# PhucNguyenAH/tacotron2_subword

Hardware: AMD Instinct MI355X
Metric: mel_frames_per_sec_train (higher is better)
Workload: dtype bf16; 1 GPU; BERT_Tacotron2 default hparams (SMA), full training iteration fwd+loss+bwd+clip+Adam, B=64/GPU, 100 phones, 60 sub-word tokens, 400 frames, 80-mel; global_batch=64, frames_per_item=400, parallelism=dp1, torch_ops=loss reductions, cat/transpose copies, persistent_chains=True, recurrent_steps_bf16=True

## Files before the change

### tacotron2_subword_amd/csrc/chain.hip

```cpp
#include <algorithm>
#include <cstdlib>
#include <type_traits>

#include "chain_common.h"

#ifdef T2_STAMPS
__device__ unsigned long long t2_chain_stamps[256 * 16];
extern "C" int t2_debug_read_chain_stamps(unsigned long long* out, int n) {
    return (int)hipMemcpyFromSymbol(out, HIP_SYMBOL(t2_chain_stamps), sizeof(unsigned long long) * n);
}
extern "C" int t2_debug_clear_chain_stamps(void) {
    static unsigned long long z[256 * 16];
    return (int)hipMemcpyToSymbol(HIP_SYMBOL(t2_chain_stamps), z, sizeof(z));
}
#define T2_CSTAMP(i)                                                                              \
    do {                                                                                          \
        __builtin_amdgcn_sched_barrier(0);                                                        \
        if (threadIdx.x == 0) { const unsigned long long n_ = __builtin_amdgcn_s_memrealtime(); t2_stamp_lds[i] += n_ - stamp_last; stamp_last = n_; } \
        __builtin_amdgcn_sched_barrier(0);                                                        \
    } while (0)
#else
#define T2_CSTAMP(i)
#endif

// ... 285 lines not shown
            }
        }
#endif
    };
    auto store_A_saved = [&](int t, int tid) {
        if (DEC) return;
#ifndef T2_CHAIN_NOSAVE
        const long rb = (long)t * B + ab_;
        for (int c = tid; c < EC; c += NTH) {
            const float x = csL[c];
            d.din[rb * d.WD + AS.coff + c0 + c] = x;
            d.dout[rb * d.WO + AS.ctx2off + c0 + c] = x;
            d.din16[rb * d.WD + AS.coff + c0 + c] = (__bf16)x;
        }
        if (KIND == CHAIN_LSA && AS.locsave) {
            const int F = d.F, DP = F + 8;
            float* ls = AS.locsave + rb * Tin * F;
            for (int i = tid; i < Tin * (F / 4); i += NTH) {
                const int j = i / (F / 4), f4 = (i % (F / 4)) * 4;
                if (j % d.CS != part) continue;
                const bf16x4 hi = *reinterpret_cast<const bf16x4*>(lspL + j * DP + f4), lo = *reinterpret_cast<const bf16x4*>(lspL + (Tin + j) * DP + f4);
                __builtin_nontemporal_store(f32x4{(float)hi[0] + (float)lo[0], (float)hi[1] + (float)lo[1], (float)hi[2] + (float)lo[2], (float)hi[3] + (float)lo[3]},
                                            reinterpret_cast<f32x4*>(ls + j * F + f4));
            }
        }
#endif
    };
#ifdef T2_STAMPS
    __shared__ __attribute__((aligned(16))) unsigned long long t2_stamp_lds[16];
    if (threadIdx.x < 16) t2_stamp_lds[threadIdx.x] = 0;
    __syncthreads();
    unsigned long long stamp_last = __builtin_amdgcn_s_memrealtime();
#endif
    for (int t = d.t0; t < d.t1; ++t) {
        const unsigned ep = (unsigned)(t - d.t0);
        const bool more = t + 1 < d.t1;
        int tv = threadIdx.x;
        asm volatile("" : "+v"(tv));
        const unsigned xout = (unsigned)((t & 1) * d.NS) * G.xs_bytes;
        if (hasL) {
            float pre[NSLOT][4];
#pragma unroll
            for (int sl = 0; sl < NSLOT; ++sl)
#pragma unroll
                for (int g = 0; g < 4; ++g) pre[sl][g] = pre_next[sl][g];
            T2_CSTAMP(15);
            if (DEC) {
                if (wave == 0 && !poll_counter(cntH_L, ep, (unsigned)G.NUG, d.err, 1u) && lane == 0) *abortw = 1;
                __syncthreads();
                if (*abortw) return;
            }
            T2_CSTAMP(0);
            if (EARLY) issue_h(t - 1);
            if (DEC) {
                if (wave == 0) {
                    bool ok = poll_counter(cntC_L, ep, nA_per_step, d.err, 2u);
                    if (ok) ok = poll_counter(d.cnt + (size_t)(10 + ls) * CNT_STRIDE, ep, (unsigned)(d.P / 16), d.err, 11u);
                    if (!ok && lane == 0) *abortw = 1;
                }
                __syncthreads();
                if (*abortw) return;
            }
            T2_CSTAMP(2);
            if (EARLY) mfma_h(t - 1);
#pragma unroll
            for (int rt = 0; rt < RT; ++rt) {
                if (!EARLY) { zero_acc(); gemm_part(t - 1, rt, wave * KH, 0, std::integral_constant<int, KH>{}); }
                if (KC > 0) gemm_part(t - 1, rt, H / 16 + wave * KC, KH, std::integral_constant<int, KC>{});
                if (DEC) gemm_part(t - 1, rt, (H + d.E) / 16 + wave * KPN, KH + KC, std::integral_constant<int, KPN>{});
                T2_CSTAMP(14);
#pragma unroll
                for (int ut = 0; ut < UT; ++ut) {
                    const int tp = rt * UT + ut;
                    if (tp > 0) __syncthreads();
#pragma unroll
                    for (int e = 0; e < 16; ++e)
                        partL[(wave * 32 + (e & 3) + 8 * (e >> 2) + 4 * hk) * PPR + r] = acc[ut][e];
                    __syncthreads();
                    if ((tid >> 8) == (tp & 1)) {
                        const int sl = tp >> 1;
                        const int bl = (tid & 255) >> 3, uu = tid & 7;
                        const int b = row0 + rt * 32 + bl, u = u0 + ut * 8 + uu;
                        float g4[4];
#pragma unroll
                        for (int g = 0; g < 4; ++g) {
                            float sum = 0.f;
#pragma unroll
                            for (int w = 0; w < NWV; ++w) sum += partL[(w * 32 + bl) * PPR + g * 8 + uu];
                            g4[g] = sum + pre[sl][g];
                        }
                        const float ig = fast_sigmoid(g4[0]), fg = fast_sigmoid(g4[1]), gg = fast_tanh(g4[2]), og = fast_sigmoid(g4[3]);
                        const float cn = fg * cst[sl] + ig * gg;
                        const float hn = og * fast_tanh(cn);
                        float ho = hn, co = cn;
                        if (d.drop_p > 0.f) {
                            const uint32_t idx = (uint32_t)(((long)t * B + b) * H + u);
                            ho = rng_keep(kh, idx, d.drop_p) ? hn * dscale : 0.f;
                            co = rng_keep(kc, idx, d.drop_p) ? cn * dscale : 0.f;
                        }
                        if (b >= B) { ho = 0.f; co = 0.f; }
                        cst[sl] = co;
                        sv[sl][0] = ig; sv[sl][1] = fg; sv[sl][2] = gg; sv[sl][3] = og; sv[sl][4] = cn; sv[sl][5] = co; sv[sl][6] = ho;
                        hsL[(rt * 32 + bl) * HSP + ut * 8 + uu] = ho;
                    }
                }
            }
            __syncthreads();
            T2_CSTAMP(3);
            if (wave < RT && rg * RT + wave < G.MT) {
                const int rtg = rg * RT + wave;
                if (UT == 2 || hk == 0) {
                    const int kh8 = UT == 2 ? hk : ((u0 >> 3) & 1);
                    const float* hp = hsL + (wave * 32 + r) * HSP + (UT == 2 ? hk * 8 : 0);
                    const f32x4 lo = *reinterpret_cast<const f32x4*>(hp), hi = *reinterpret_cast<const f32x4*>(hp + 4);
                    bf16x8 o;
#pragma unroll
                    for (int j = 0; j < 4; ++j) { o[j] = (__bf16)lo[j]; o[4 + j] = (__bf16)hi[j]; }
                    u32x4 ow = __builtin_bit_cast(u32x4, o);
                    if (!DEC) ow.x = (ow.x & ~1u) | step_tag(t);
                    __builtin_amdgcn_raw_buffer_store_b128(ow, rsX,
                        xout + (unsigned)ls * G.xs_bytes + (unsigned)((((u0 >> 4) * G.MT + rtg) * 64 + kh8 * 32 + r) * 16), 0, SC1);
                }
            }
            if (KIND != CHAIN_LSTM) {
                if (wave < 4 * RT) {
                    const int ct = wave & 3, rt = wave >> 2;
                    f32x16 qa;
#pragma unroll
                    for (int e = 0; e < 16; ++e) qa[e] = 0.f;
#pragma unroll
                    for (int m = 0; m < UT * 4; ++m)
                        qa = __builtin_amdgcn_mfma_f32_32x32x2f32(hsL[(rt * 32 + r) * HSP + 2 * m + hk], wqf[m], qa, 0, 0, 0);
#pragma unroll
                    for (int e = 0; e < 16; ++e) qsL[(rt * 32 + (e & 3) + 8 * (e >> 2) + 4 * hk) * (A + 4) + ct * 32 + r] = qa[e];
                }
                __syncthreads();
                const unsigned qb = (unsigned)(((ls * G.NRG + rg) * G.NUG + ug) * (32 * RT)) * (unsigned)(A * 4);
                for (int i = tv; i < RT * 32 * (A / 4); i += NTH) {
                    const int row = i / (A / 4), a4 = (i % (A / 4)) * 4;
                    const f32x4 v4 = *reinterpret_cast<const f32x4*>(qsL + row * (A + 4) + a4);
                    u32x4 vw = __builtin_bit_cast(u32x4, v4);
                    vw.x = (vw.x & ~1u) | tag_q(t);
                    __builtin_amdgcn_raw_buffer_store_b128(vw, rsQ, qb + (unsigned)((row * A + a4) * 4), 0, SC1);
                }
            }
            T2_CSTAMP(4);
            if (DEC) publish(cntH_L, (unsigned)ug); else { __syncthreads(); if (*abortw) return; }
            T2_CSTAMP(5);
            store_L_saved(t, tv);
            if (!DEC && !hasA && more) load_pre(t + 1, tv);
        }
        if (hasA) {
            const int tid = tv, lane = tid & 63, wave = tid >> 6;
            T2_CSTAMP(6);
            if (KIND == CHAIN_LSA) {
                const int F = d.F, Kc = d.Kc, pad = (Kc - 1) / 2, Tw = Tin + Kc - 1, TwP = (Tw + 8 + 3) & ~3, KP = (Kc + 7) & ~7, WP = 2 * KP + 8;
                for (int i = tid; i < 2 * TwP; i += NTH) {
                    const int c = i / TwP, j = i % TwP - pad;
                    wpadL[i] = (j >= 0 && j < Tin) ? (c == 0 ? apL[j] : cumL[j]) : 0.f;
                }
                __syncthreads();
                const int r_ = lane & 31, h_ = lane >> 5;
                const int njt = (Tin + 31) / 32, nft = (F + 31) / 32;
                for (int tile = wave; tile < njt * nft; tile += NWV) {
                    const int jt = tile / nft, ft = tile % nft;
                    const float* xr = wpadL + min(jt * 32 + r_, Tin - 1);
                    const __bf16* wh = convwL + min(ft * 32 + r_, F - 1) * WP + 8 * h_;
                    f32x16 acc;
#pragma unroll
                    for (int e2 = 0; e2 < 16; ++e2) acc[e2] = 0.f;
                    for (int k0 = 0; k0 < 2 * KP; k0 += 16) {
                        const int ck = k0 + 8 * h_, c = ck >= KP ? 1 : 0;
                        const float* xp = xr + c * TwP + ck - c * KP;
                        float xv[8];
#pragma unroll
                        for (int u = 0; u < 8; ++u) xv[u] = xp[u];
                        bf16x8 ah, al;
#pragma unroll
                        for (int u = 0; u < 8; ++u) { ah[u] = (__bf16)xv[u]; al[u] = (__bf16)(xv[u] - (float)ah[u]); }
                        const bf16x8 bh = *reinterpret_cast<const bf16x8*>(wh + k0), bl = *reinterpret_cast<const bf16x8*>(wh + F * WP + k0);
                        acc = __builtin_amdgcn_mfma_f32_32x32x16_bf16(al, bh, acc, 0, 0, 0);
                        acc = __builtin_amdgcn_mfma_f32_32x32x16_bf16(ah, bl, acc, 0, 0, 0);
                        acc = __builtin_amdgcn_mfma_f32_32x32x16_bf16(ah, bh, acc, 0, 0, 0);
                    }
                    const int f = ft * 32 + r_;
                    if (f < F) {
#pragma unroll
                        for (int e2 = 0; e2 < 16; ++e2) {
                            const int row = jt * 32 + (e2 & 3) + 8 * (e2 >> 2) + 4 * h_;
                            if (row < Tin) {
                                const float x = acc[e2];
                                const __bf16 hi = (__bf16)x;
                                lspL[row * (F + 8) + f] = hi; lspL[(Tin + row) * (F + 8) + f] = (__bf16)(x - (float)hi);
                            }
                        }
                    }
                }
            }
            if (KIND == CHAIN_LSA) __syncthreads();
            if (*abortw) return;
            T2_CSTAMP(7);
            {
                const int pg = tid >> 5, a4 = (tid & 31) * 4;
                const unsigned qb = (unsigned)((as * G.NRG + arg) * G.NUG) * (unsigned)(32 * RT * A * 4) + (unsigned)((arow * A + a4) * 4);
                constexpr int QU = 4;
                u32x4 pv[QU];
                auto load_q = [&](int i0) {
                    const unsigned long long tsp = __builtin_amdgcn_s_memrealtime();
                    for (;;) {
                        unsigned okw = 1u;
#pragma unroll
                        for (int k = 0; k < QU; ++k) {
                            pv[k] = __builtin_amdgcn_raw_buffer_load_b128(rsQ, qb + (unsigned)min(i0 + 16 * k, G.NUG - 1) * (unsigned)(32 * RT * A * 4), 0, SC1);
                            okw &= ((pv[k].x & 1u) == tag_q(t)) ? 1u : 0u;
                        }
                        if (__all(okw != 0u)) break;
                        if (__builtin_amdgcn_s_memrealtime() - tsp > SPIN_TICKS) { if ((tid & 63) == 0) { report_abort(d.err, 19u); *abortw = 1; } break; }
                    }
                };
                load_q(pg);
                f32x4 accq = {0.f, 0.f, 0.f, 0.f};
#pragma unroll
                for (int k = 0; k < QU; ++k) if (pg + 16 * k < G.NUG) accq += __builtin_bit_cast(f32x4, pv[k]);
                for (int i0 = pg + 16 * QU; i0 < G.NUG; i0 += 16 * QU) {
                    load_q(i0);
#pragma unroll
                    for (int k = 0; k < QU; ++k) if (i0 + 16 * k < G.NUG) accq += __builtin_bit_cast(f32x4, pv[k]);
                }
                *reinterpret_cast<f32x4*>(redL + pg * A + a4) = accq;
                if (!DEC && more) load_pre(t + 1, tid);
            }
            __syncthreads();
            if (tid < A) {
                float sum = 0.f;
#pragma unroll
                for (int k = 0; k < 16; ++k) sum += redL[k * A + tid];
                qL[tid] = sum;
                if (!DEC && part == 0) AS.qs[((long)t * B + ab_) * A + tid] = sum;
            }
            __syncthreads();
            T2_CSTAMP(8);
            if (KIND == CHAIN_LSA) {
                const int njt = (Tin + 31) / 32, nat = A / 32, TinP = (Tin + 3) & ~3;
                const int r_ = lane & 31, h_ = lane >> 5;
                constexpr float K2 = 2.0f * 1.44269504088896341f;
                for (int tile = wave; tile < njt * nat; tile += NWV) {
                    const int jt = tile % njt, at = tile / njt;
                    const int j = min(jt * 32 + r_, Tin - 1);
                    const int DP = d.F + 8;
                    const __bf16* dh = denseL + (at * 32 + r_) * DP + 8 * h_;
                    const __bf16* lh = lspL + j * DP + 8 * h_;
                    f32x16 acc;
#pragma unroll
                    for (int e2 = 0; e2 < 16; ++e2) acc[e2] = 0.f;
                    for (int k0 = 0; k0 < d.F; k0 += 16) {
                        const bf16x8 ah = *reinterpret_cast<const bf16x8*>(dh + k0), al = *reinterpret_cast<const bf16x8*>(dh + A * DP + k0);
                        const bf16x8 bh = *reinterpret_cast<const bf16x8*>(lh + k0), bl = *reinterpret_cast<const bf16x8*>(lh + Tin * DP + k0);
                        acc = __builtin_amdgcn_mfma_f32_32x32x16_bf16(al, bh, acc, 0, 0, 0);
                        acc = __builtin_amdgcn_mfma_f32_32x32x16_bf16(ah, bl, acc, 0, 0, 0);
                        acc = __builtin_amdgcn_mfma_f32_32x32x16_bf16(ah, bh, acc, 0, 0, 0);
                    }
                    const float* pr = pmL + j * (A + 1) + at * 32 + 4 * h_;
                    const float* qr = qL + at * 32 + 4 * h_;
                    const float* vr = vL + at * 32 + 4 * h_;
                    float sum = 0.f;
                    float* up = (!DEC && AS.usave && (tile / NWV + wave) % d.CS == part && jt * 32 + r_ < Tin)
                                    ? AS.usave + (((long)t * B + ab_) * A + at * 32 + 4 * h_) * TinP + j : nullptr;
#pragma unroll
                    for (int e2 = 0; e2 < 16; ++e2) {
                        const int ao = (e2 & 3) + 8 * (e2 >> 2);
                        const float x = qr[ao] + pr[ao] + acc[e2];
                        const float sg = __builtin_amdgcn_rcpf(__builtin_amdgcn_exp2f(K2 * x) + 1.0f);
                        sum += vr[ao] * sg;
                        if (up) __builtin_nontemporal_store(1.0f - 2.0f * sg, up + ao * TinP);
                    }
                    sum += __shfl_xor(sum, 32, 64);
                    if (h_ == 0 && jt * 32 + r_ < Tin) paL[at * Tp + jt * 32 + r_] = sum;
                }
                __syncthreads();
                for (int jj = tid; jj < Tin; jj += NTH) {
                    float sum = 0.f;
                    for (int at = 0; at < nat; ++at) sum += paL[at * Tp + jj];
                    eL[jj] = vL[A] - 2.0f * sum;
                }
            } else {
            {
                const int gid = tid >> 4, sub = tid & 15;
                f32x4 qv[2], vv[2];
                float vsum = 0.f;
#pragma unroll
                for (int k = 0; k < 2; ++k) {
                    qv[k] = *reinterpret_cast<const f32x4*>(qL + sub * 4 + 64 * k);
                    vv[k] = *reinterpret_cast<const f32x4*>(vL + sub * 4 + 64 * k);
                    qv[k] *= 2.0f * 1.44269504088896341f;
                    vsum += (vv[k][0] + vv[k][1]) + (vv[k][2] + vv[k][3]);
                }
                constexpr float K2 = 2.0f * 1.44269504088896341f;
                auto dot = [&](f32x4 (&pv)[2], int j) {
                    float sum = 0.f;
#pragma unroll
                    for (int k = 0; k < 2; ++k)
#pragma unroll
                        for (int c = 0; c < 4; ++c)
                            sum += vv[k][c] * __builtin_amdgcn_rcpf(__builtin_amdgcn_exp2f(fmaf(pv[k][c], K2, qv[k][c])) + 1.0f);
                    return vsum - 2.0f * sum;
                };
                auto finish = [&](int j, float s0) {
                    s0 += __shfl_xor(s0, 8, 64); s0 += __shfl_xor(s0, 4, 64);
                    s0 += __shfl_xor(s0, 2, 64); s0 += __shfl_xor(s0, 1, 64);
                    if (sub == 0) eL[j] = s0;
                };
                const int nres = min(Jp, Tin);
                int j = gid;
                for (; j < nres; j += 2 * (NTH / 16)) {
                    const int j1 = j + NTH / 16;
                    f32x4 p0[2], p1[2];
#pragma unroll
                    for (int k = 0; k < 2; ++k) {
                        p0[k] = *reinterpret_cast<const f32x4*>(pmL + j * A + sub * 4 + 64 * k);
                        p1[k] = *reinterpret_cast<const f32x4*>(pmL + min(j1, nres - 1) * A + sub * 4 + 64 * k);
                    }
                    finish(j, dot(p0, j));
                    if (j1 < nres) finish(j1, dot(p1, min(j1, nres - 1)));
                }
                for (j = nres + gid; j < Tin; j += NTH / 16) {
                    const float* pr = AS.pm + ((long)ab_ * Tin + j) * A + sub * 4;
                    f32x4 p0[2];
#pragma unroll
                    for (int k = 0; k < 2; ++k) p0[k] = *reinterpret_cast<const f32x4*>(pr + 64 * k);
                    finish(j, dot(p0, j));
                }
            }
            }
            __syncthreads();
            T2_CSTAMP(9);
            if (KIND == CHAIN_SMA) {
                float maskv = AS.mask_value;
                asm volatile("" : "+v"(maskv));
                for (int j = tid; j < Tin; j += NTH) {
                    float ev = eL[j];
                    if (j >= alen) ev = maskv;
                    if (d.noise_std > 0.f) ev += d.noise_std * rng_normal(kn, (uint32_t)(((long)t * B + ab_) * Tin + j));
                    const float p = fast_sigmoid(ev);
                    eL[j] = p;
                    if (!DEC && part == 0) AS.psel[((long)ab_ * d.T + t) * Tin + j] = p;
                }
                __syncthreads();
                for (int j = tid; j < Tin; j += NTH) {
                    float a = apL[j] * eL[j];
                    if (j > 0) a += apL[j - 1] * (1.0f - eL[j - 1]);
                    anL[j] = a;
                    if (part == 0) AS.align[((long)ab_ * d.T + t) * Tin + j] = a;
                }
            } else {
                float maskv = AS.mask_value;
                asm volatile("" : "+v"(maskv));
                float mx = -INFINITY;
                for (int j = tid; j < Tin; j += NTH) {
                    float ev = eL[j];
                    if (j >= alen) ev = maskv;
                    eL[j] = ev;
                    mx = fmaxf(mx, ev);
                }
                mx = wave_max(mx);
                if (lane == 0) credL[wave] = mx;
                __syncthreads();
                mx = credL[0];
#pragma unroll
                for (int w = 1; w < NWV; ++w) mx = fmaxf(mx, credL[w]);
                float sum = 0.f;
                for (int j = tid; j < Tin; j += NTH) { const float x = __expf(eL[j] - mx); eL[j] = x; sum += x; }
                sum = wave_sum(sum);
                __syncthreads();
                if (lane == 0) credL[wave] = sum;
                __syncthreads();
                sum = credL[0];
#pragma unroll
                for (int w = 1; w < NWV; ++w) sum += credL[w];
                const float inv = 1.0f / sum;
                for (int j = tid; j < Tin; j += NTH) {
                    const float w = eL[j] * inv;
                    anL[j] = w;
                    const float cm = cumL[j] + w;
                    cumL[j] = cm;
                    if (part == 0) {
                        AS.align[((long)ab_ * d.T + t) * Tin + j] = w;
                        AS.wcum[((long)ab_ * d.T + t) * Tin + j] = cm;
                    }
                }
            }
            __syncthreads();
            T2_CSTAMP(10);
            {
                const int ncl = EC / 4, nres = min(Jm, Tin);
                for (int cb = 0; cb < ncl; cb += 64) {
                    const int cl = cb + lane;
                    if (cl < ncl) {
                        f32x4 accc = {0.f, 0.f, 0.f, 0.f};
#pragma unroll 4
                        for (int j = wave; j < nres; j += NWV) {
                            const bf16x4 mb = *reinterpret_cast<const bf16x4*>(memL + j * EC + cl * 4);
                            accc += anL[j] * f32x4{(float)mb[0], (float)mb[1], (float)mb[2], (float)mb[3]};
                        }
#pragma unroll 4
                        for (int j = nres + wave; j < Tin; j += NWV)
                            accc += anL[j] * *reinterpret_cast<const f32x4*>(AS.memory + ((long)ab_ * Tin + j) * d.E + c0 + cl * 4);
                        *reinterpret_cast<f32x4*>(credL + wave * EC + cl * 4) = accc;
                    }
                }
            }
            __syncthreads();
            for (int c = tid; c < EC; c += NTH) {
                float sum = 0.f;
#pragma unroll
                for (int w = 0; w < NWV; ++w) sum += credL[w * EC + c];
                csL[c] = sum;
            }
            for (int j = tid; j < Tin; j += NTH) apL[j] = anL[j];
            __syncthreads();
            if (tid < EC / 8) {
                const int pc = c0 / 8 + tid;
                const f32x4 lo = *reinterpret_cast<const f32x4*>(csL + tid * 8), hi = *reinterpret_cast<const f32x4*>(csL + tid * 8 + 4);
                bf16x8 o;
#pragma unroll
                for (int j = 0; j < 4; ++j) { o[j] = (__bf16)lo[j]; o[4 + j] = (__bf16)hi[j]; }
                const int kt = H / 16 + pc / 2;
                u32x4 ow = __builtin_bit_cast(u32x4, o);
                if (!DEC) ow.x = (ow.x & ~1u) | step_tag(t);
                __builtin_amdgcn_raw_buffer_store_b128(ow, rsX,
                    xout + (unsigned)as * G.xs_bytes + (unsigned)(((kt * G.MT + ab_ / 32) * 64 + (pc & 1) * 32 + (ab_ & 31)) * 16), 0, SC1);
            }
            T2_CSTAMP(11);
            if (DEC) publish(cntC_A, (unsigned)(arow * d.CS + part)); else { __syncthreads(); if (*abortw) return; }
            T2_CSTAMP(12);
            store_A_saved(t, tid);
        }
        if (DEC) {
            const int tid = tv, lane = tid & 63, wave = tid >> 6, r = lane & 31, hk = lane >> 5;
            const int j16 = lane & 15, kq = lane >> 4;
            const unsigned xcur = (unsigned)((t & 1) * d.NS) * G.xs_bytes;
            unsigned* cntD = d.cnt + (size_t)8 * CNT_STRIDE;
            unsigned* cntM = d.cnt + (size_t)9 * CNT_STRIDE;
            T2_CSTAMP(13);
            if (hasD) {
                {
                    const int kgw = wave * (DNW * 32), sg0 = H + Ee, sg1 = 2 * (H + Ee);
                    const bool fd = kgw >= sg1;
                    const int stw = kgw < sg0 ? 0 : 1;
                    const bool isc = !fd && kgw - stw * sg0 >= H;
                    const unsigned* cp = fd ? cntD : d.cnt + (size_t)(2 * stw + (isc ? 1 : 0)) * CNT_STRIDE;
                    const unsigned wsteps = fd ? ep : ep + 1, wprod = fd ? (unsigned)(Hd / DU) : isc ? (unsigned)(B * d.CS) : (unsigned)G.NUG;
                    if (!poll_counter(cp, wsteps, wprod, d.err, 12u) && lane == 0) *abortw = 1;
                }
                T2_CSTAMP(1);
                const int kg = wave * (DNW * 32);
                const int seg0 = H + Ee, seg1 = 2 * (H + Ee);
                const bool from_d = kg >= seg1;
                const int st = kg < seg0 ? 0 : 1;
                const int lk = from_d ? kg - seg1 : kg - st * seg0;
                const unsigned base = from_d ? (unsigned)(((t + 1) & 1) * (Hd / 16) * 1024) : xcur + (unsigned)st * G.xs_bytes;
                f32x4 accd[2] = {{0.f, 0.f, 0.f, 0.f}, {0.f, 0.f, 0.f, 0.f}};
#pragma unroll
                for (int i0 = 0; i0 < DNW; i0 += 4) {
                    u32x4 af[4][2];
#pragma unroll
                    for (int i = 0; i < 4; ++i)
#pragma unroll
                        for (int m = 0; m < 2; ++m)
                            af[i][m] = from_d ? __builtin_amdgcn_raw_buffer_load_b128(rsD, base + frag16(lane, lk + (i0 + i) * 32, m), 0, SC1)
                                              : __builtin_amdgcn_raw_buffer_load_b128(rsX, base + frag16(lane, lk + (i0 + i) * 32, m), 0, SC1);
#pragma unroll
                    for (int i = 0; i < 4; ++i)
#pragma unroll
                        for (int m = 0; m < 2; ++m)
                            accd[m] = __builtin_amdgcn_mfma_f32_16x16x32_bf16(__builtin_bit_cast(bf16x8, af[i][m]), WD[i0 + i], accd[m], 0, 0, 0);
                }
#pragma unroll
                for (int m = 0; m < 2; ++m)
#pragma unroll
                    for (int e = 0; e < 4; ++e) partDL[(wave * 32 + m * 16 + kq * 4 + e) * 20 + j16] = accd[m][e];
                __syncthreads();
                if (*abortw) return;
                if (tid < 32 * DU) {
                    const int row = tid >> 2, uu = tid & 3;
                    float g4[4];
#pragma unroll
                    for (int g = 0; g < 4; ++g) {
                        float sum = 0.f;
#pragma unroll
                        for (int w = 0; w < NWV; ++w) sum += partDL[(w * 32 + row) * 20 + g * 4 + uu];
                        g4[g] = sum + dbias[g];
                    }
                    const float ig = fast_sigmoid(g4[0]), fg = fast_sigmoid(g4[1]), gg = fast_tanh(g4[2]), og = fast_sigmoid(g4[3]);
                    const float cn = fg * dcst + ig * gg;
                    dcst = cn;
                    stgL[row * 20 + uu] = row < B ? og * fast_tanh(cn) : 0.f;
                    if (t == d.t1 - 1 && row < B) d.dec_c[(long)row * Hd + du0 + uu] = cn;
                }
                __syncthreads();
                if (tid < 32) {
                    const f32x4 h4 = *reinterpret_cast<const f32x4*>(stgL + tid * 20);
                    bf16x4 o; o[0] = (__bf16)h4[0]; o[1] = (__bf16)h4[1]; o[2] = (__bf16)h4[2]; o[3] = (__bf16)h4[3];
                    typedef unsigned int u32x2 __attribute__((ext_vector_type(2)));
                    __builtin_amdgcn_raw_buffer_store_b64(__builtin_bit_cast(u32x2, o), rsD,
                        (unsigned)((t & 1) * (Hd / 16) * 1024) + (unsigned)((((du0 >> 4) * 64) + ((du0 >> 3) & 1) * 32 + tid) * 16 + ((du0 & 7) >> 2) * 8), 0, SC1);
                }
                T2_CSTAMP(6);
                publish(cntD, (unsigned)wg);
            }
            if (hasP1) {
                const int kg = wave * 256;
                const bool from_d = kg < Hd;
                const int st = kg < Hd + Ee ? 0 : 1;
                if (!poll_counter(from_d ? cntD : d.cnt + (size_t)(2 * st + 1) * CNT_STRIDE,
                                  ep + 1, from_d ? (unsigned)(Hd / DU) : (unsigned)(B * d.CS), d.err, 13u) && lane == 0) *abortw = 1;
                const int lk = from_d ? kg : H + (kg - Hd - st * Ee);
                const unsigned base = from_d ? (unsigned)((t & 1) * (Hd / 16) * 1024) : xcur + (unsigned)st * G.xs_bytes;
                f32x4 accp[2] = {{0.f, 0.f, 0.f, 0.f}, {0.f, 0.f, 0.f, 0.f}};
#pragma unroll
                for (int i0 = 0; i0 < 8; i0 += 4) {
                    u32x4 af[4][2];
#pragma unroll
                    for (int i = 0; i < 4; ++i)
#pragma unroll
                        for (int m = 0; m < 2; ++m)
                            af[i][m] = from_d ? __builtin_amdgcn_raw_buffer_load_b128(rsD, base + frag16(lane, lk + (i0 + i) * 32, m), 0, SC1)
                                              : __builtin_amdgcn_raw_buffer_load_b128(rsX, base + frag16(lane, lk + (i0 + i) * 32, m), 0, SC1);
#pragma unroll
                    for (int i = 0; i < 4; ++i) {
                        const bf16x8 wb = wfragL[(wave * 8 + i0 + i) * 64 + lane];
#pragma unroll
                        for (int m = 0; m < 2; ++m)
                            accp[m] = __builtin_amdgcn_mfma_f32_16x16x32_bf16(__builtin_bit_cast(bf16x8, af[i][m]), wb, accp[m], 0, 0, 0);
                    }
                }
#pragma unroll
                for (int m = 0; m < 2; ++m)
#pragma unroll
                    for (int e = 0; e < 4; ++e) partDL[(wave * 32 + m * 16 + kq * 4 + e) * 20 + j16] = accp[m][e];
                __syncthreads();
                if (*abortw) return;
                {
                    const int row = tid >> 4, col = p1g * 16 + (tid & 15);
                    float sum = 0.f;
#pragma unroll
                    for (int w = 0; w < NWV; ++w) sum += partDL[(w * 32 + row) * 20 + (tid & 15)];
                    float val = 0.f;
                    if (col < Mm) {
                        val = sum + d.proj_b[col];
                        if (row < B) d.mel_out[(long)row * d.ldmel + (long)t * Mm + col] = val;
                    } else if (col == Mm && row < B) {
                        const float gt = sum + d.gate_b[0];
                        d.gate_out[(long)row * d.ldgate + t] = gt;
                        if (d.stop_index && d.stop_index[row] < 0 && 1.0f / (1.0f + expf(-gt)) > d.thr) { d.stop_index[row] = t; atomicAdd(d.done, 1); }
                    }
                    stgL[row * 20 + (tid & 15)] = (col < Mm && row < B) ? val : 0.f;
                }
                __syncthreads();
                if (wave == 0) {
                    const float* hp = stgL + r * 20 + hk * 8;
                    const f32x4 lo = *reinterpret_cast<const f32x4*>(hp), hi = *reinterpret_cast<const f32x4*>(hp + 4);
                    bf16x8 o;
#pragma unroll
                    for (int j = 0; j < 4; ++j) { o[j] = (__bf16)lo[j]; o[4 + j] = (__bf16)hi[j]; }
                    __builtin_amdgcn_raw_buffer_store_b128(__builtin_bit_cast(u32x4, o), rsM, (unsigned)(((t & 1) * 8 + p1g) * 1024 + lane * 16), 0, SC1);
                }
                publish(cntM, (unsigned)p1g);
            }
            if (hasP2 && t + 1 < d.T) {
                if (wave == 0 && !poll_counter(cntM, ep + 1, (unsigned)((Mm + 1 + 15) / 16), d.err, 14u) && lane == 0) *abortw = 1;
                __syncthreads();
                if (*abortw) return;
                const RngKey k1 = rng_key(d.seed, d.psite1[p2s]), k2 = rng_key(d.seed, d.psite2[p2s]);
                const float pscale = d.pdrop > 0.f ? 1.0f / (1.0f - d.pdrop) : 1.0f;
                const uint32_t ibase = (uint32_t)((long)(t + 1) * B * Pn);
// ... 110 lines not shown
```

### tacotron2_subword_amd/csrc/chain_bwd.hip

```cpp
#include <algorithm>

#include "chain_common.h"

#ifdef T2_STAMPS
__device__ unsigned long long t2_chain_bwd_stamps[256 * 16];
extern "C" int t2_debug_read_chain_bwd_stamps(unsigned long long* out, int n) {
    return (int)hipMemcpyFromSymbol(out, HIP_SYMBOL(t2_chain_bwd_stamps), sizeof(unsigned long long) * n);
}
extern "C" int t2_debug_clear_chain_bwd_stamps(void) {
    static unsigned long long z[256 * 16];
    return (int)hipMemcpyToSymbol(HIP_SYMBOL(t2_chain_bwd_stamps), z, sizeof(z));
}
#define T2_BSTAMP(i)                                                                              \
    do {                                                                                          \
        __builtin_amdgcn_sched_barrier(0);                                                        \
        if (threadIdx.x == 0) { const unsigned long long n_ = __builtin_amdgcn_s_memrealtime(); t2_stamp_lds[i] += n_ - stamp_last; stamp_last = n_; } \
        __builtin_amdgcn_sched_barrier(0);                                                        \
    } while (0)
#else
#define T2_BSTAMP(i)
#endif

namespace t2 {

// ... 246 lines not shown

    if (tid == 0) *abortw = 0;

    bf16x8 W[16];
    if (hasG) {
#pragma unroll
        for (int i = 0; i < 16; ++i)
            W[i] = KIND == CHAIN_LSA
                       ? *reinterpret_cast<const bf16x8*>(GS.wt16 + (long)(nt * ANC + (i >> 3) * 32 + r) * GS.ldwt + kp * H + (wave * 8 + (i & 7)) * 16 + 8 * hk)
                       : *reinterpret_cast<const bf16x8*>(GS.wt16 + (long)(nt * ANC + (wave & 1) * 32 + r) * GS.ldwt + kp * H + ((wave >> 1) * 16 + i) * 16 + 8 * hk);
    }
    const int pb = rt * 32 + (tid >> 4), pu = u0 + (tid & 15);
    float dc = 0.f;
    float bacc[4] = {0.f, 0.f, 0.f, 0.f};
    float pin[7];
    auto load_pin = [&](int t, int tid) {
        const int b = min(rt * 32 + (tid >> 4), B - 1), u = u0 + (tid & 15);
        const long rb = (long)t * B + b;
        pin[0] = PS.dh1[rb * PS.lddh1 + u];
        const float* gp = PS.gates + rb * K4 + u;
        pin[1] = gp[0]; pin[2] = gp[H]; pin[3] = gp[2 * H]; pin[4] = gp[3 * H];
        pin[5] = PS.c_new[rb * H + u];
        pin[6] = t > 0 ? PS.c_out[((long)(t - 1) * B + b) * H + u] : 0.f;
    };
    if (hasP) {
        for (int i = tid; i < A * PU; i += NTH) {
            const float x = PS.wq[(long)(i / PU) * H + u0 + i % PU];
            const __bf16 hi = (__bf16)x;
            wq16L[(i % PU) * (A + 8) + i / PU] = hi; wq16L[(PU + i % PU) * (A + 8) + i / PU] = (__bf16)(x - (float)hi);
        }
        load_pin(d.t1 - 1, tid);
    }
    const int F = d.F, Kc = d.Kc, F1 = F + 1, pad = (Kc - 1) / 2, TwP = M.TwP, UP = A + 4, WN = len + 2 * pad;
    const int CP = (2 * Kc + 15) & ~15;
    float* wL = smem + M.ps;
    float* ccL = smem + M.cc; float* convwL = smem + M.convw; float* dlocL = smem + M.dloc; float* wpadL = smem + M.wpad;
    float* utL = smem + M.scratch + M.ut; float* locL = smem + M.scratch + M.loc; float* lredL = smem + M.scratch + M.red;
    (void)F1; (void)TwP; (void)UP; (void)WN; (void)CP; (void)wL; (void)ccL; (void)convwL; (void)dlocL; (void)wpadL; (void)utL; (void)locL; (void)lredL;
    auto pack8 = [&](auto f) {
        bf16x8 o;
#pragma unroll
        for (int i = 0; i < 8; ++i) o[i] = (__bf16)f(i);
        return o;
    };
    auto mfma_chain = [&](int n, auto fa, auto fb, f32x16 acc) {
        f32x16 acc2;
#pragma unroll
        for (int e = 0; e < 16; ++e) acc2[e] = 0.f;
        for (int i0 = 0; i0 < n; i0 += 8) {
            float av[8], bv[8];
#pragma unroll
            for (int u = 0; u < 8; ++u) { av[u] = fa(i0 + u); bv[u] = fb(i0 + u); }
            __builtin_amdgcn_sched_barrier(0);
#pragma unroll
            for (int u = 0; u < 8; u += 2) {
                acc = __builtin_amdgcn_mfma_f32_32x32x2f32(av[u], bv[u], acc, 0, 0, 0);
                acc2 = __builtin_amdgcn_mfma_f32_32x32x2f32(av[u + 1], bv[u + 1], acc2, 0, 0, 0);
            }
            __builtin_amdgcn_sched_barrier(0);
        }
#pragma unroll
        for (int e = 0; e < 16; ++e) acc[e] += acc2[e];
        return acc;
    };
    f32x16 accWd, accWc;
#pragma unroll
    for (int e = 0; e < 16; ++e) { accWd[e] = 0.f; accWc[e] = 0.f; }
    float ain[6];
    auto load_ain = [&](int t, int tid) {
        const long rb = (long)t * B + ab_;
        ain[0] = (KIND != CHAIN_LSA && tid < A) ? AS.qs[rb * A + tid] : 0.f;
        const int j = jb + tid;
        const bool in = tid < ng;
        if constexpr (KIND == CHAIN_LSA) {
            ain[1] = tid < len ? AS.align[((long)ab_ * d.T + t) * Tin + j] : 0.f;
            const int c = tid / WN, x = tid - c * WN, jw = jb - pad + x;
            ain[2] = (tid < 2 * WN && t > 0 && jw >= 0 && jw < Tin) ? (c == 0 ? AS.align : AS.wcum)[((long)ab_ * d.T + t - 1) * Tin + jw] : 0.f;
        } else {
            ain[1] = (in && tid < len) ? AS.psel[((long)ab_ * d.T + t) * Tin + j] : 0.f;
            ain[2] = (in && tid < len) ? (t > 0 ? AS.align[((long)ab_ * d.T + t - 1) * Tin + j] : (j == 0 ? 1.f : 0.f)) : 0.f;
        }
        ain[3] = (in && AS.dalign) ? AS.dalign[((long)ab_ * d.T + t) * Tin + j] : 0.f;
        ain[4] = tid < E ? AS.dctx_a[rb * AS.lddctx_a + tid] : 0.f;
        ain[5] = tid < E ? AS.dctx_b[rb * AS.lddctx_b + tid] : 0.f;
    };
    if (hasA) {
        for (int a = tid; a < A; a += NTH) { vL[a] = AS.v[a]; dvaL[a] = 0.f; }
        for (int i = tid; i < len * (A / 4); i += NTH) {
            const int jl = i / (A / 4), a4 = (i % (A / 4)) * 4;
            if constexpr (KIND == CHAIN_SMA)
                *reinterpret_cast<f32x4*>(pmL + jl * A + a4) = *reinterpret_cast<const f32x4*>(AS.pm + ((long)ab_ * Tin + jb + jl) * A + a4);
            *reinterpret_cast<f32x4*>(dpmL + jl * A + a4) = f32x4{0.f, 0.f, 0.f, 0.f};
        }
        for (int i = tid; i < ng * (E / 4); i += NTH) {
            const int jl = i / (E / 4), c4 = (i % (E / 4)) * 4;
            const f32x4 m4 = *reinterpret_cast<const f32x4*>(AS.memory + ((long)ab_ * Tin + jb + jl) * E + c4);
            bf16x4 o; o[0] = (__bf16)m4[0]; o[1] = (__bf16)m4[1]; o[2] = (__bf16)m4[2]; o[3] = (__bf16)m4[3];
            *reinterpret_cast<bf16x4*>(memL + jl * E + c4) = o;
        }
        for (int j = tid; j < chunk + 8; j += NTH) carryL[j] = 0.f;
        if constexpr (KIND == CHAIN_LSA) {
            for (int j = tid; j < chunk + 8; j += NTH) ccL[j] = 0.f;
            for (int i = tid; i < F * CP; i += NTH) { const int f = i / CP, ck = i - f * CP; convwL[i] = ck < 2 * Kc ? AS.loc_conv[f * 2 * Kc + ck] : 0.f; }
            for (int i = tid; i < (d.lds_Tc + 2 * pad) * F1; i += NTH) dlocL[i] = 0.f;
            for (int i = tid; i < 4 * TwP; i += NTH) wpadL[i] = 0.f;
        }
        load_ain(d.t1 - 1, tid);
    }
    __syncthreads();
    const RngKey kh = rng_key(d.seed, PS.site_h), kc = rng_key(d.seed, PS.site_c);
    const float dscale = d.drop_p > 0.f ? 1.0f / (1.0f - d.drop_p) : 1.0f;

#ifdef T2_STAMPS
    __shared__ __attribute__((aligned(16))) unsigned long long t2_stamp_lds[16];
    if (threadIdx.x < 16) t2_stamp_lds[threadIdx.x] = 0;
    __syncthreads();
    unsigned long long stamp_last = __builtin_amdgcn_s_memrealtime();
#endif
    for (int t = d.t1 - 1; t >= d.t0; --t) {
        const unsigned ep = (unsigned)(d.t1 - 1 - t);
        int tv = threadIdx.x;
        asm volatile("" : "+v"(tv));
        if (hasA) {
            if constexpr (KIND == CHAIN_SMA) {
            const int tid = tv, lane = tid & 63, wave = tid >> 6;
            T2_BSTAMP(15);
            float in[6];
#pragma unroll
            for (int i = 0; i < 6; ++i) in[i] = ain[i];
            T2_BSTAMP(0);
            float boundary = 0.f;
            if (tid < E) {
                float v = in[4] + in[5];
                if (ep > 0) {
                    const unsigned off = (unsigned)((t + 1) & 1) * pbc_half + (unsigned)as * pbc_s + (unsigned)((ab_ * E + tid) * 4);
                    float pv[AKP];
                    load_tagged4(rsC, off, pbc_kp, step_tag(ep - 1), pv, 7u);
                    v += (pv[0] + pv[1]) + (pv[2] + pv[3]);
                }
                dctxL[tid] = v;
                if (split == 0) AS.dctx_out[((long)t * B + ab_) * E + tid] = v;
            }
            if (tid == 0 && ep > 0 && je < Tin) {
                const unsigned long long tsp = __builtin_amdgcn_s_memrealtime();
                for (;;) {
                    const unsigned wv = __builtin_amdgcn_raw_buffer_load_b32(rsK, (unsigned)((((t + 1) & 1) * d.NS + as) * B + ab_) * 4u, 0, SC1);
                    boundary = __builtin_bit_cast(float, wv);
                    if ((wv & 1u) == step_tag(ep - 1)) break;
                    if (__builtin_amdgcn_s_memrealtime() - tsp > SPIN_TICKS) { report_abort(d.err, 14u); *abortw = 1; break; }
                }
            }
            if (tid < A) qL[tid] = in[0];
            if (tid < len) { psL[tid] = in[1]; apL[tid] = in[2]; }
            if (tid == 0) { gL[ng] = 0.f; if (je < Tin) carryL[len] = boundary; }
            __syncthreads();
            if (*abortw) return;
            T2_BSTAMP(1);
            for (int jl = wave; jl < ng; jl += NWV) {
                float sum = 0.f;
                for (int c = lane * 8; c < E; c += 512) {
                    const bf16x8 mb = *reinterpret_cast<const bf16x8*>(memL + jl * E + c);
                    const f32x4 d0 = *reinterpret_cast<const f32x4*>(dctxL + c), d1 = *reinterpret_cast<const f32x4*>(dctxL + c + 4);
#pragma unroll
                    for (int k = 0; k < 4; ++k) sum += (float)mb[k] * d0[k] + (float)mb[4 + k] * d1[k];
                }
                sum = wave_sum(sum);
                if (lane == 0) {
                    float gsum = sum;
                    gL[jl] = gsum;
                }
            }
            __syncthreads();
            if (tid < ng) {
                float gsum = gL[tid] + in[3];
                if (ep > 0) gsum += carryL[tid];
                gL[tid] = gsum;
            }
            __syncthreads();
            if (tid < len) {
                const float p = psL[tid], gj = gL[tid], gn = gL[tid + 1];
                deL[tid] = apL[tid] * (gj - gn) * p * (1.0f - p);
                const float co = gj * p + gn * (1.0f - p);
                carryL[tid] = co;
                if (tid == 0 && split == 1)
                    __builtin_amdgcn_raw_buffer_store_b32(__builtin_bit_cast(unsigned, tag_f32(co, step_tag(ep))), rsK, (unsigned)(((t & 1) * d.NS + as) * B + ab_) * 4u, 0, SC1);
            }
            __syncthreads();
            T2_BSTAMP(2);
            {
                const int gid = tid >> 4, sub = tid & 15;
                f32x4 dq[2], dv[2];
#pragma unroll
                for (int k = 0; k < 2; ++k) { dq[k] = f32x4{0.f, 0.f, 0.f, 0.f}; dv[k] = f32x4{0.f, 0.f, 0.f, 0.f}; }
                for (int jl = gid; jl < len; jl += NTH / 16) {
                    const float dej = deL[jl];
#pragma unroll
                    for (int k = 0; k < 2; ++k) {
                        const int a = sub * 4 + 64 * k;
                        const f32x4 pv = *reinterpret_cast<const f32x4*>(pmL + jl * A + a);
                        f32x4 acc = *reinterpret_cast<const f32x4*>(dpmL + jl * A + a);
#pragma unroll
                        for (int c = 0; c < 4; ++c) {
                            const float u = fast_tanh(qL[a + c] + pv[c]);
                            const float dpre = dej * vL[a + c] * (1.0f - u * u);
                            dq[k][c] += dpre; dv[k][c] += dej * u; acc[c] += dpre;
                        }
                        *reinterpret_cast<f32x4*>(dpmL + jl * A + a) = acc;
                    }
                }
#pragma unroll
                for (int k = 0; k < 2; ++k)
#pragma unroll
                    for (int c = 0; c < 4; ++c) {
                        dq[k][c] += __shfl_xor(dq[k][c], 16, 64); dq[k][c] += __shfl_xor(dq[k][c], 32, 64);
                        dv[k][c] += __shfl_xor(dv[k][c], 16, 64); dv[k][c] += __shfl_xor(dv[k][c], 32, 64);
                    }
                if (lane < 16) {
#pragma unroll
                    for (int k = 0; k < 2; ++k) {
                        *reinterpret_cast<f32x4*>(redL + wave * A + sub * 4 + 64 * k) = dq[k];
                        *reinterpret_cast<f32x4*>(redL + (NWV + wave) * A + sub * 4 + 64 * k) = dv[k];
                    }
                }
            }
            __syncthreads();
            if (tid < A) {
                float sq = 0.f, sv = 0.f;
#pragma unroll
                for (int k = 0; k < NWV; ++k) { sq += redL[k * A + tid]; sv += redL[(NWV + k) * A + tid]; }
                dqoL[tid] = sq;
                dvaL[tid] += sv;
            }
            __syncthreads();
            if (tid < A / 4) {
                const f32x4 q4 = *reinterpret_cast<const f32x4*>(dqoL + tid * 4);
                u32x4 qw = __builtin_bit_cast(u32x4, q4);
                qw.x = (qw.x & ~1u) | ((ep & 1u) ^ 1u);
                __builtin_amdgcn_raw_buffer_store_b128(qw, rsQ, (unsigned)((((as * 2 + split) * B + ab_) * A + tid * 4) * 4), 0, SC1);
            }
            T2_BSTAMP(3);
            __syncthreads();
            T2_BSTAMP(4);
            if (tid < A) AS.dq_out[((long)t * B + ab_) * 2 * A + split * A + tid] = dqoL[tid];
            if (t > d.t0) load_ain(t - 1, tid);
                    } else {
            const int tid = tv, lane = tid & 63, wave = tid >> 6, r = lane & 31, hk = lane >> 5;
            T2_BSTAMP(15);
            float in[6];
#pragma unroll
            for (int i = 0; i < 6; ++i) in[i] = ain[i];
            float* wnew = wpadL + (t & 1) * 2 * TwP;
            const float* wold = wpadL + ((t + 1) & 1) * 2 * TwP;
            const int njt = (len + 31) / 32;
            if (ep > 0 && tid < pad * (F / 4) && ((split == 0 && je < Tin) || (split == 1 && jb > 0))) {
                const int row = tid / (F / 4), f4 = (tid % (F / 4)) * 4;
                const unsigned off = (unsigned)((((((t + 1) & 1) * d.NS + as) * B + ab_) * 2 + (1 - split)) * pad * F + row * F + f4) * 4u;
                u32x4 hw;
                const unsigned long long tsp = __builtin_amdgcn_s_memrealtime();
                for (;;) {
                    hw = __builtin_amdgcn_raw_buffer_load_b128(rsK, off, 0, SC1);
                    if ((hw.x & 1u) == step_tag(ep - 1)) break;
                    if (__builtin_amdgcn_s_memrealtime() - tsp > SPIN_TICKS) { report_abort(d.err, 11u); *abortw = 1; break; }
                }
                const f32x4 h4 = __builtin_bit_cast(f32x4, hw);
                float* dst = dlocL + (split == 0 ? len + pad + row : row) * F1 + f4;
                dst[0] = h4[0]; dst[1] = h4[1]; dst[2] = h4[2]; dst[3] = h4[3];
            }
            f32x4 ureg[4], lreg;
            const int TinP = (Tin + 3) & ~3, nj4 = (len + 3) >> 2;
            {
                const float* us = AS.usave + ((long)t * B + ab_) * A * TinP + jb;
#pragma unroll
                for (int k = 0; k < 4; ++k) {
                    const int w = wave + NWV * k, a = (w & 7) * 16 + (lane & 15), j4 = min((w >> 3) * 4 + (lane >> 4), nj4 - 1);
                    ureg[k] = *reinterpret_cast<const f32x4*>(us + (long)a * TinP + 4 * j4);
                }
                const int i = min(tid, len * (F / 4) - 1);
                lreg = *reinterpret_cast<const f32x4*>(AS.locsave + (((long)t * B + ab_) * Tin + jb + i / (F / 4)) * F + (i % (F / 4)) * 4);
            }
            if (tid < len) wL[tid] = in[1];
            if (tid < 2 * WN) { const int c = tid / WN; wnew[c * TwP + (tid - c * WN)] = in[2]; }
            __syncthreads();
            T2_BSTAMP(11);
            if (ep > 0) {
                const int NP = len + 2 * pad, qi = wave < 2 ? wave : wave - 2, pt = qi >> 1, nq = qi & 1;
                if ((wave < 2 || wave >= 4) && pt * 32 < NP && nq * 32 < 2 * Kc) {
                    const float* ar = dlocL + min(pt * 32 + r, NP - 1) * F1 + 8 * hk;
                    const float* br = convwL + 8 * hk * CP + min(nq * 32 + r, 2 * Kc - 1);
                    f32x16 acc;
#pragma unroll
                    for (int e = 0; e < 16; ++e) acc[e] = 0.f;
#pragma unroll
                    for (int ks = 0; ks < 2; ++ks)
                        acc = __builtin_amdgcn_mfma_f32_32x32x16_bf16(pack8([&](int i) { return ar[16 * ks + i]; }),
                                                                        pack8([&](int i) { return br[(16 * ks + i) * CP]; }), acc, 0, 0, 0);
                    const int n = nq * 32 + r;
                    if (n < 2 * Kc) {
#pragma unroll
                        for (int e = 0; e < 16; ++e) {
                            const int p = pt * 32 + (e & 3) + 8 * (e >> 2) + 4 * hk;
                            if (p < NP) utL[p * 65 + n] = acc[e];
                        }
                    }
                }
                if ((wave == 2 || wave == 3) && (wave - 2) * 32 < 2 * Kc) {
                    const int n = min((wave - 2) * 32 + r, 2 * Kc - 1), c = n / Kc, k = n - c * Kc;
                    const float* ar = dlocL + pad * F1 + min(r, F);
                    const float* br = wold + c * TwP + k;
                    for (int ks = 0; ks * 16 < len; ++ks) {
                        const int j0 = ks * 16 + 8 * hk;
                        accWc = __builtin_amdgcn_mfma_f32_32x32x16_bf16(
                            pack8([&](int i) { const float x = ar[min(j0 + i, len - 1) * F1]; return j0 + i < len ? x : 0.f; }),
                            pack8([&](int i) { return br[min(j0 + i, len - 1)]; }), accWc, 0, 0, 0);
                    }
                }
            }
            __syncthreads();
            T2_BSTAMP(12);
            if (ep > 0 && tid < 2 * len) {
                const int c = tid / len, i = tid - c * len;
                const float* qp = utL + (i + 2 * pad) * 65 + c * Kc;
                float sum = 0.f;
                for (int k = 0; k < Kc; ++k) sum += qp[-k * 64];
                if (c == 0) carryL[i] = sum; else ccL[i] += sum;
            }
            __syncthreads();
#pragma unroll
            for (int k = 0; k < 4; ++k) {
                const int w = wave + NWV * k, a = (w & 7) * 16 + (lane & 15), j4 = (w >> 3) * 4 + (lane >> 4);
#pragma unroll
                for (int c = 0; c < 4; ++c)
                    if (4 * j4 + c < len) utL[(4 * j4 + c) * UP + a] = ureg[k][c];
            }
            if (tid < len * (F / 4)) {
                float* lw = locL + (tid / (F / 4)) * F1 + (tid % (F / 4)) * 4;
                lw[0] = lreg[0]; lw[1] = lreg[1]; lw[2] = lreg[2]; lw[3] = lreg[3];
            }
            if (tid < len) locL[tid * F1 + F] = 0.f;
            T2_BSTAMP(13);
            __syncthreads();
            if (*abortw) return;
            T2_BSTAMP(0);
            if (tid < E) {
                float v = in[4] + in[5];
                if (ep > 0) {
                    const unsigned off = (unsigned)((t + 1) & 1) * pbc_half + (unsigned)as * pbc_s + (unsigned)((ab_ * E + tid) * 4);
                    float pv[AKP];
                    load_tagged4(rsC, off, pbc_kp, step_tag(ep - 1), pv, 7u);
                    v += (pv[0] + pv[1]) + (pv[2] + pv[3]);
                }
                dctxL[tid] = v;
                if (split == 0) AS.dctx_out[((long)t * B + ab_) * E + tid] = v;
            }
            __syncthreads();
            T2_BSTAMP(1);
            for (int jl = wave; jl < len; jl += NWV) {
                float sum = 0.f;
                for (int c = lane * 8; c < E; c += 512) {
                    const bf16x8 mb = *reinterpret_cast<const bf16x8*>(memL + jl * E + c);
                    const f32x4 d0 = *reinterpret_cast<const f32x4*>(dctxL + c), d1 = *reinterpret_cast<const f32x4*>(dctxL + c + 4);
#pragma unroll
                    for (int k = 0; k < 4; ++k) sum += (float)mb[k] * d0[k] + (float)mb[4 + k] * d1[k];
                }
                sum = wave_sum(sum);
                if (lane == 0) gL[jl] = sum;
            }
            __syncthreads();
            float part = 0.f;
            if (tid < len) {
                float gsum = gL[tid] + in[3];
                if (ep > 0) gsum += carryL[tid] + ccL[tid];
                gL[tid] = gsum;
                part = wL[tid] * gsum;
            }
            part = wave_sum(part);
            if (lane == 0) lredL[wave] = part;
            __syncthreads();
            if (wave == 0) {
                float mine = 0.f;
#pragma unroll
                for (int w = 0; w < NWV; ++w) mine += lredL[w];
                const unsigned sbase = (unsigned)(pad * F * 2 * d.NS * B * 2) * 4u;
                const unsigned soff = sbase + (unsigned)((((t & 1) * d.NS + as) * B + ab_) * 2) * 8u;
                typedef unsigned int u32x2 __attribute__((ext_vector_type(2)));
                if (lane == 0) {
                    u32x2 o; o[0] = __builtin_bit_cast(unsigned, mine); o[1] = (unsigned)(t + 1);
                    __builtin_amdgcn_raw_buffer_store_b64(o, rsK, soff + (unsigned)split * 8u, 0, SC1);
                }
// ... 413 lines not shown
```

Measured before the change: 1.065 million mel-frames/s.

## Remove barriers in attention chain step via fused sigmoid and ping-pong alignment buffers

In the forward chain, the SMA sigmoid, masking and noise are folded into the energy reduction's finish step. The alignment buffers now ping-pong by step parity, so the copy from the new to the previous alignment and one barrier go away, and the context partial sums are reduced directly in the store stage. In the backward chain, the per-position gradient dot products are batched four per wave with fused reductions and carry adds, and the dq/dv reductions are split across thread ranges to drop a barrier. The aim is fewer __syncthreads and serial phases per recurrent step, at the cost of more register pressure and extra RNG precompute into cumL.

```diff
diff --git a/tacotron2_subword_amd/csrc/chain.hip b/tacotron2_subword_amd/csrc/chain.hip
--- a/tacotron2_subword_amd/csrc/chain.hip
+++ b/tacotron2_subword_amd/csrc/chain.hip
@@ -461,12 +461,14 @@
         }
         if (hasA) {
             const int tid = tv, lane = tid & 63, wave = tid >> 6;
+            const float* apC = smem + ((ep & 1u) ? M.an : M.ap);
+            float* anC = smem + ((ep & 1u) ? M.ap : M.an);
             T2_CSTAMP(6);
             if (KIND == CHAIN_LSA) {
                 const int F = d.F, Kc = d.Kc, pad = (Kc - 1) / 2, Tw = Tin + Kc - 1, TwP = (Tw + 8 + 3) & ~3, KP = (Kc + 7) & ~7, WP = 2 * KP + 8;
                 for (int i = tid; i < 2 * TwP; i += NTH) {
                     const int c = i / TwP, j = i % TwP - pad;
-                    wpadL[i] = (j >= 0 && j < Tin) ? (c == 0 ? apL[j] : cumL[j]) : 0.f;
+                    wpadL[i] = (j >= 0 && j < Tin) ? (c == 0 ? apC[j] : cumL[j]) : 0.f;
                 }
                 __syncthreads();
                 const int r_ = lane & 31, h_ = lane >> 5;
@@ -508,6 +510,8 @@
             }
             if (KIND == CHAIN_LSA) __syncthreads();
             if (*abortw) return;
+            if (KIND == CHAIN_SMA && d.noise_std > 0.f)
+                for (int j = tid; j < Tin; j += NTH) cumL[j] = rng_normal(kn, (uint32_t)(((long)t * B + ab_) * Tin + j));
             T2_CSTAMP(7);
             {
                 const int pg = tid >> 5, a4 = (tid & 31) * 4;
@@ -614,10 +618,19 @@
                             sum += vv[k][c] * __builtin_amdgcn_rcpf(__builtin_amdgcn_exp2f(fmaf(pv[k][c], K2, qv[k][c])) + 1.0f);
                     return vsum - 2.0f * sum;
                 };
+                float maskv = AS.mask_value;
+                asm volatile("" : "+v"(maskv));
                 auto finish = [&](int j, float s0) {
                     s0 += __shfl_xor(s0, 8, 64); s0 += __shfl_xor(s0, 4, 64);
                     s0 += __shfl_xor(s0, 2, 64); s0 += __shfl_xor(s0, 1, 64);
-                    if (sub == 0) eL[j] = s0;
+                    if (sub == 0) {
+                        float ev = s0;
+                        if (j >= alen) ev = maskv;
+                        if (d.noise_std > 0.f) ev = fmaf(d.noise_std, cumL[j], ev);
+                        const float p = fast_sigmoid(ev);
+                        eL[j] = p;
+                        if (!DEC && part == 0) AS.psel[((long)ab_ * d.T + t) * Tin + j] = p;
+                    }
                 };
                 const int nres = min(Jp, Tin);
                 int j = gid;
@@ -644,21 +657,10 @@
             __syncthreads();
             T2_CSTAMP(9);
             if (KIND == CHAIN_SMA) {
-                float maskv = AS.mask_value;
-                asm volatile("" : "+v"(maskv));
                 for (int j = tid; j < Tin; j += NTH) {
-                    float ev = eL[j];
-                    if (j >= alen) ev = maskv;
-                    if (d.noise_std > 0.f) ev += d.noise_std * rng_normal(kn, (uint32_t)(((long)t * B + ab_) * Tin + j));
-                    const float p = fast_sigmoid(ev);
-                    eL[j] = p;
-                    if (!DEC && part == 0) AS.psel[((long)ab_ * d.T + t) * Tin + j] = p;
-                }
-                __syncthreads();
-                for (int j = tid; j < Tin; j += NTH) {
-                    float a = apL[j] * eL[j];
-                    if (j > 0) a += apL[j - 1] * (1.0f - eL[j - 1]);
-                    anL[j] = a;
+                    float a = apC[j] * eL[j];
+                    if (j > 0) a += apC[j - 1] * (1.0f - eL[j - 1]);
+                    anC[j] = a;
                     if (part == 0) AS.align[((long)ab_ * d.T + t) * Tin + j] = a;
                 }
             } else {
@@ -689,7 +691,7 @@
                 const float inv = 1.0f / sum;
                 for (int j = tid; j < Tin; j += NTH) {
                     const float w = eL[j] * inv;
-                    anL[j] = w;
+                    anC[j] = w;
                     const float cm = cumL[j] + w;
                     cumL[j] = cm;
                     if (part == 0) {
@@ -709,27 +711,25 @@
 #pragma unroll 4
                         for (int j = wave; j < nres; j += NWV) {
                             const bf16x4 mb = *reinterpret_cast<const bf16x4*>(memL + j * EC + cl * 4);
-                            accc += anL[j] * f32x4{(float)mb[0], (float)mb[1], (float)mb[2], (float)mb[3]};
+                            accc += anC[j] * f32x4{(float)mb[0], (float)mb[1], (float)mb[2], (float)mb[3]};
                         }
 #pragma unroll 4
                         for (int j = nres + wave; j < Tin; j += NWV)
-                            accc += anL[j] * *reinterpret_cast<const f32x4*>(AS.memory + ((long)ab_ * Tin + j) * d.E + c0 + cl * 4);
+                            accc += anC[j] * *reinterpret_cast<const f32x4*>(AS.memory + ((long)ab_ * Tin + j) * d.E + c0 + cl * 4);
                         *reinterpret_cast<f32x4*>(credL + wave * EC + cl * 4) = accc;
                     }
                 }
             }
-            __syncthreads();
-            for (int c = tid; c < EC; c += NTH) {
-                float sum = 0.f;
-#pragma unroll
-                for (int w = 0; w < NWV; ++w) sum += credL[w * EC + c];
-                csL[c] = sum;
-            }
-            for (int j = tid; j < Tin; j += NTH) apL[j] = anL[j];
             __syncthreads();
             if (tid < EC / 8) {
                 const int pc = c0 / 8 + tid;
-                const f32x4 lo = *reinterpret_cast<const f32x4*>(csL + tid * 8), hi = *reinterpret_cast<const f32x4*>(csL + tid * 8 + 4);
+                f32x4 lo = {0.f, 0.f, 0.f, 0.f}, hi = {0.f, 0.f, 0.f, 0.f};
+#pragma unroll
+                for (int w = 0; w < NWV; ++w) {
+                    lo += *reinterpret_cast<const f32x4*>(credL + w * EC + tid * 8);
+                    hi += *reinterpret_cast<const f32x4*>(credL + w * EC + tid * 8 + 4);
+                }
+                *reinterpret_cast<f32x4*>(csL + tid * 8) = lo; *reinterpret_cast<f32x4*>(csL + tid * 8 + 4) = hi;
                 bf16x8 o;
 #pragma unroll
                 for (int j = 0; j < 4; ++j) { o[j] = (__bf16)lo[j]; o[4 + j] = (__bf16)hi[j]; }
diff --git a/tacotron2_subword_amd/csrc/chain_bwd.hip b/tacotron2_subword_amd/csrc/chain_bwd.hip
--- a/tacotron2_subword_amd/csrc/chain_bwd.hip
+++ b/tacotron2_subword_amd/csrc/chain_bwd.hip
@@ -422,29 +422,40 @@
             }
             if (tid < A) qL[tid] = in[0];
             if (tid < len) { psL[tid] = in[1]; apL[tid] = in[2]; }
+            if (tid < ng) deL[tid] = in[3];
             if (tid == 0) { gL[ng] = 0.f; if (je < Tin) carryL[len] = boundary; }
             __syncthreads();
             if (*abortw) return;
             T2_BSTAMP(1);
-            for (int jl = wave; jl < ng; jl += NWV) {
-                float sum = 0.f;
-                for (int c = lane * 8; c < E; c += 512) {
-                    const bf16x8 mb = *reinterpret_cast<const bf16x8*>(memL + jl * E + c);
-                    const f32x4 d0 = *reinterpret_cast<const f32x4*>(dctxL + c), d1 = *reinterpret_cast<const f32x4*>(dctxL + c + 4);
-#pragma unroll
-                    for (int k = 0; k < 4; ++k) sum += (float)mb[k] * d0[k] + (float)mb[4 + k] * d1[k];
-                }
-                sum = wave_sum(sum);
-                if (lane == 0) {
-                    float gsum = sum;
-                    gL[jl] = gsum;
-                }
-            }
-            __syncthreads();
-            if (tid < ng) {
-                float gsum = gL[tid] + in[3];
-                if (ep > 0) gsum += carryL[tid];
-                gL[tid] = gsum;
+            {
+                constexpr int GP = 4;
+                for (int j0 = wave; j0 < ng; j0 += GP * NWV) {
+                    float sum[GP], da[GP], cy[GP];
+#pragma unroll
+                    for (int q = 0; q < GP; ++q) {
+                        const int jl = min(j0 + q * NWV, ng - 1);
+                        da[q] = deL[jl]; cy[q] = carryL[jl];
+                        sum[q] = 0.f;
+                        for (int c = lane * 8; c < E; c += 512) {
+                            const bf16x8 mb = *reinterpret_cast<const bf16x8*>(memL + jl * E + c);
+                            const f32x4 d0 = *reinterpret_cast<const f32x4*>(dctxL + c), d1 = *reinterpret_cast<const f32x4*>(dctxL + c + 4);
+#pragma unroll
+                            for (int k = 0; k < 4; ++k) sum[q] += (float)mb[k] * d0[k] + (float)mb[4 + k] * d1[k];
+                        }
+                    }
+#pragma unroll
+                    for (int o = 32; o > 0; o >>= 1)
+#pragma unroll
+                        for (int q = 0; q < GP; ++q) sum[q] += __shfl_xor(sum[q], o, 64);
+                    if (lane == 0) {
+#pragma unroll
+                        for (int q = 0; q < GP; ++q) {
+                            float gsum = sum[q] + da[q];
+                            if (ep > 0) gsum += cy[q];
+                            if (j0 + q * NWV < ng) gL[j0 + q * NWV] = gsum;
+                        }
+                    }
+                }
             }
             __syncthreads();
             if (tid < len) {
@@ -494,16 +505,17 @@
                 }
             }
             __syncthreads();
-            if (tid < A) {
-                float sq = 0.f, sv = 0.f;
-#pragma unroll
-                for (int k = 0; k < NWV; ++k) { sq += redL[k * A + tid]; sv += redL[(NWV + k) * A + tid]; }
-                dqoL[tid] = sq;
-                dvaL[tid] += sv;
-            }
-            __syncthreads();
+            if (tid >= 64 && tid < 64 + A) {
+                float sv = 0.f;
+#pragma unroll
+                for (int k = 0; k < NWV; ++k) sv += redL[(NWV + k) * A + tid - 64];
+                dvaL[tid - 64] += sv;
+            }
             if (tid < A / 4) {
-                const f32x4 q4 = *reinterpret_cast<const f32x4*>(dqoL + tid * 4);
+                f32x4 q4 = {0.f, 0.f, 0.f, 0.f};
+#pragma unroll
+                for (int k = 0; k < NWV; ++k) q4 += *reinterpret_cast<const f32x4*>(redL + k * A + tid * 4);
+                *reinterpret_cast<f32x4*>(dqoL + tid * 4) = q4;
                 u32x4 qw = __builtin_bit_cast(u32x4, q4);
                 qw.x = (qw.x & ~1u) | ((ep & 1u) ^ 1u);
                 __builtin_amdgcn_raw_buffer_store_b128(qw, rsQ, (unsigned)((((as * 2 + split) * B + ab_) * A + tid * 4) * 4), 0, SC1);
```

Result: no change. 1.070 million mel-frames/s (median of 6 runs) (+0.5%).
